# IGLICT/NeRFFaceEditing

Hardware: NVIDIA B200
Metric: rendered rays/sec (48+48 samples) (higher is better)
Workload: dtype f32 (gather, compositing) + bf16x3 split tensor-core MLP with f32 accumulate

## Files before the change

### include/nfe_b200.h

```cpp
#ifndef NFE_B200_H
#define NFE_B200_H

#include <stdint.h>

#ifdef __cplusplus
extern "C" {
#endif

typedef void* nfe_stream_t;

int nfe_version(void);
const char* nfe_last_error(void);
uint64_t nfe_launch_count(void);
int nfe_timing_enable(int on);
int nfe_timing_read(double* ms_by_stage, int64_t* count_by_stage, int n_stages, int reset);

int nfe_bench_l2_gather(const float* table, int64_t n_lines, int warps_per_cta, int depth, int iters, int64_t* host_lines_out,
                        float* sink, nfe_stream_t stream);

int nfe_plane_stats(const float* planes, int64_t n_slabs, int64_t hw, float* mean, float* std_out,
                    nfe_stream_t stream);
int nfe_plane_normalize(const float* planes, const float* mean, const float* std_in, int64_t n_slabs,
                        int64_t hw, float* out, nfe_stream_t stream);
int nfe_plane_denormalize(const float* norm, const float* mean, const float* std_in, int64_t n_slabs,
                          int64_t stat_slabs, int64_t hw, float* out, nfe_stream_t stream);
int nfe_plane_normalize_bwd(const float* g_norm, const float* norm, const float* std_in, const float* g_mean,
                            const float* g_std, int64_t n_slabs, int64_t hw, double* sums_ws, float* g_planes,
                            nfe_stream_t stream);
int nfe_resize_bilinear(const float* in, int64_t n_img, int in_h, int in_w, int out_h, int out_w, int antialias,
                        float* out, nfe_stream_t stream);
int nfe_planes_to_channel_last(const float* planes, int64_t n_img, int channels, int64_t hw, float* out,
                               nfe_stream_t stream);

int nfe_plane_normalize_staged(const float* planes, const float* mean, const float* std_in, int64_t n_img,
                               int64_t hw, float* out_norm, float* out_norm_cl, float* out_raw_cl,
                               nfe_stream_t stream);

int nfe_generate_rays(const float* cam2world , const float* intrinsics , int n,
                      int resolution, float* origins , float* dirs, nfe_stream_t stream);
int nfe_ray_limits_box(const float* origins, const float* dirs, int64_t n_rays, float box_side_length,
                       float* tmin, float* tmax, nfe_stream_t stream);

int nfe_sample_stratified(int64_t n_rays, int s_c, int mode, const float* table, double ray_start,
                          double ray_end, const float* start_per_ray, const float* end_per_ray,
                          const float* jitter, int stochastic, uint64_t seed, uint64_t offset,
                          float* depths , nfe_stream_t stream);

int nfe_sample_planes_fwd(const float* planes_cl, int plane_batch, int channels, int height, int width,
                          const float* coords , int n, int64_t m, float box_warp, float* out,
                          nfe_stream_t stream);

// ... 144 lines not shown
```

### nerffaceediting_b200/_lib.py

```python
import ctypes
import os

_HERE = os.path.dirname(os.path.abspath(__file__))
LIB_PATH = os.path.join(_HERE, "lib", "libnfe_b200.so")

DEC_OSG, DEC_DISENTANGLED, DEC_SEGMENTATION = 0, 1, 2
PREC_FP32, PREC_BF16X3, PREC_BF16 = 0, 1, 2

c_f32p = ctypes.c_void_p
c_i64 = ctypes.c_int64
c_u64 = ctypes.c_uint64
c_int = ctypes.c_int
c_float = ctypes.c_float
c_double = ctypes.c_double
c_vp = ctypes.c_void_p


class NfeMlp(ctypes.Structure):
    _fields_ = [("w1", c_vp), ("b1", c_vp), ("w2", c_vp), ("b2", c_vp),
                ("in_dim", c_int), ("hidden", c_int), ("out_dim", c_int),
                ("wgain1", c_float), ("bgain1", c_float), ("wgain2", c_float), ("bgain2", c_float)]


class NfeRenderCfg(ctypes.Structure):
# ... 12 lines not shown


_MLP_P = ctypes.POINTER(NfeMlp)
_CFG_P = ctypes.POINTER(NfeRenderCfg)

SIGNATURES = {
    "nfe_version": (c_int, []),
    "nfe_last_error": (ctypes.c_char_p, []),
    "nfe_launch_count": (c_u64, []),
    "nfe_timing_enable": (c_int, [c_int]),
    "nfe_timing_read": (c_int, [ctypes.POINTER(c_double), ctypes.POINTER(c_i64), c_int, c_int]),
    "nfe_bench_l2_gather": (c_int, [c_vp, c_i64, c_int, c_int, c_int, ctypes.POINTER(c_i64), c_vp, c_vp]),
    "nfe_plane_stats": (c_int, [c_vp, c_i64, c_i64, c_vp, c_vp, c_vp]),
    "nfe_plane_normalize": (c_int, [c_vp, c_vp, c_vp, c_i64, c_i64, c_vp, c_vp]),
    "nfe_plane_denormalize": (c_int, [c_vp, c_vp, c_vp, c_i64, c_i64, c_i64, c_vp, c_vp]),
    "nfe_plane_normalize_staged": (c_int, [c_vp, c_vp, c_vp, c_i64, c_i64, c_vp, c_vp, c_vp, c_vp]),
    "nfe_planes_to_channel_last": (c_int, [c_vp, c_i64, c_int, c_i64, c_vp, c_vp]),
    "nfe_generate_rays": (c_int, [c_vp, c_vp, c_int, c_int, c_vp, c_vp, c_vp]),
    "nfe_ray_limits_box": (c_int, [c_vp, c_vp, c_i64, c_float, c_vp, c_vp, c_vp]),
    "nfe_sample_stratified": (c_int, [c_i64, c_int, c_int, c_vp, c_double, c_double, c_vp, c_vp, c_vp, c_int, c_u64, c_u64, c_vp, c_vp]),
    "nfe_sample_planes_fwd": (c_int, [c_vp, c_int, c_int, c_int, c_int, c_vp, c_int, c_i64, c_float, c_vp, c_vp]),
    "nfe_decoder_fwd": (c_int, [c_int, c_int, _MLP_P, _MLP_P, c_vp, c_vp, c_int, c_i64, c_int, c_vp, c_vp, c_vp, c_vp]),
    "nfe_composite_fwd": (c_int, [c_vp, c_vp, c_vp, c_vp, c_i64, c_int, c_int, c_int, c_int, c_vp, c_vp, c_vp, c_vp, c_vp, c_vp, c_vp]),
    "nfe_importance_resample": (c_int, [c_vp, c_vp, c_i64, c_int, c_int, c_vp, c_int, c_u64, c_u64, c_vp, c_vp, c_vp, c_vp]),
    "nfe_sample_pdf": (c_int, [c_vp, c_vp, c_i64, c_int, c_int, c_int, c_vp, c_int, c_u64, c_u64, c_float, c_vp, c_vp]),
    "nfe_unify_samples":(c_int, [c_vp] * 8 + [c_i64, c_int, c_int, c_int, c_int] + [c_vp] * 4 + [c_vp]),
    "nfe_render_workspace_bytes": (c_i64, [_CFG_P, c_int, c_i64]),
    "nfe_render_fwd": (c_int, [_CFG_P, _MLP_P, _MLP_P, c_vp, c_vp, c_int, c_vp, c_vp, c_int, c_i64, c_vp, c_vp,
                               c_vp, c_vp, c_vp, c_vp, c_vp, c_int, c_vp, c_vp, c_vp, c_i64, c_vp]),
    "nfe_render_workspace_layout": (c_int, [_CFG_P, c_int, c_i64, ctypes.POINTER(c_i64)]),
    "nfe_composite_bwd": (c_int, [c_vp, c_vp, c_vp, c_int, c_vp, c_vp, c_vp, c_int, c_i64, c_int, c_int, c_vp, c_vp, c_vp, c_vp, c_vp, c_vp, c_vp, c_vp]),
# ... 66 lines not shown
```

### nerffaceediting_b200/autograd.py

```python
import ctypes
import os

import torch
import torch.nn.functional as F

from . import _lib, ops

MAX_ROWS = 1 << 22


def _mlp(x, seq):
    a, b = seq[0], seq[2]
    h = F.softplus(torch.addmm((a.bias * a.bias_gain).unsqueeze(0), x, (a.weight * a.weight_gain).t()))
    return torch.addmm((b.bias * b.bias_gain).unsqueeze(0), h, (b.weight * b.weight_gain).t())


def _decode(kind, seq_a, seq_b, fn, fd):
    if kind == ops.DEC_DISENTANGLED:
        g = _mlp(fn, seq_a)
        return g[:, :1], g[:, 1:], torch.sigmoid(_mlp(fd, seq_b)) * (1 + 2 * 0.001) - 0.001
    x = _mlp(fd, seq_a)
    rgb = torch.sigmoid(x[:, 1:]) * (1 + 2 * 0.001) - 0.001
    return x[:, :1], (_mlp(fd, seq_b) if kind == ops.DEC_SEGMENTATION else None), rgb

# ... 210 lines not shown
        if g.get("rgb") is not None:
            g_rec[:, 16:48] = g["rgb"].reshape(n * m, 32)
        with torch.cuda.device(dev):
            fb = _FieldBackward(kind, seq_a, seq_b, norm_cl, denorm_cl, ctx.affine, ctx.box_warp, ctx.needs_input_grad[5:], dev)
            fb.run_pass(n, rec, g_rec, coords=coords)
            norm_shape, plane_shape = ctx.plane_shapes
            g_norm, g_planes, g_scale, g_shift, g_params = fb.finish(norm_shape, plane_shape, ctx.needs_input_grad[1], ctx.needs_input_grad[2],
                                                                     ctx.stat_shapes, ctx.needs_input_grad[3], ctx.needs_input_grad[4])
        return (None, g_norm, g_planes, g_scale, g_shift) + tuple(g_params)


class NormalizeFunction(torch.autograd.Function):

    @staticmethod
    def forward(ctx, planes):
        mean, std = ops.plane_stats(planes)
        norm_cl = None
        if planes.dim() == 4 and planes.shape[1] == 96 and planes.is_contiguous() and planes.dtype == torch.float32:
            norm, norm_cl, _ = ops.plane_normalize_staged(planes.detach(), mean, std, register=False)
        else:
            norm = ops.plane_normalize(planes, mean, std)
        ctx.save_for_backward(norm, std)
        ctx.hw = planes.shape[-1] * planes.shape[-2]
        if norm_cl is None:
            return norm, mean, std, None
        ctx.mark_non_differentiable(norm_cl)
        return norm, mean, std, norm_cl

    @staticmethod
    def backward(ctx, g_norm, g_mean, g_std, _g_cl=None):
        norm, std = ctx.saved_tensors
        def f32(t):
            return None if t is None else t.contiguous().float()
        g, gm, gs = f32(g_norm), f32(g_mean), f32(g_std)
        slabs = norm.numel() // ctx.hw
# ... 30 lines not shown
```

### nerffaceediting_b200/csrc/nfe_march.cu

```cuda
#include "nfe_march.cuh"

namespace nfe {

__device__ __forceinline__ double shfl_up_double(double v, int delta)
{
    int lo = __double2loint(v), hi = __double2hiint(v);
    lo = __shfl_up_sync(0xffffffffu, lo, delta);
    hi = __shfl_up_sync(0xffffffffu, hi, delta);
    return __hiloint2double(hi, lo);
}
__device__ __forceinline__ double shfl_xor_double(double v, int mask)
{
    int lo = __double2loint(v), hi = __double2hiint(v);
    lo = __shfl_xor_sync(0xffffffffu, lo, mask);
    hi = __shfl_xor_sync(0xffffffffu, hi, mask);
    return __hiloint2double(hi, lo);
}

__device__ __forceinline__ void ray_interval_weights(const float* s_depth, const float* s_sigma, float* s_w, int S, int lane, float& wd, float& wt)
{
    const int n_int = S - 1;
    const int chunk = (n_int + 31) / 32;
    const int i0 = lane * chunk, i1 = min(n_int, i0 + chunk);
    float prod = 1.0f;
    for (int i = i0; i < i1; ++i) {
        const float delta = __fsub_rn(s_depth[i + 1], s_depth[i]);
        const float sig = __fdiv_rn(__fadd_rn(s_sigma[i], s_sigma[i + 1]), 2.0f);
        const float xs = __fsub_rn(sig, 1.0f);
        const float dens = fmaxf(xs, 0.0f) + __logf(1.0f + __expf(-fabsf(xs)));
        const float alpha = __fsub_rn(1.0f, __expf(-__fmul_rn(dens, delta)));
        s_w[i] = alpha;
        prod *= __fadd_rn(__fsub_rn(1.0f, alpha), 1e-10f);
    }
    float incl = prod;
#pragma unroll
    for (int o = 1; o < 32; o <<= 1) {
        const float up = __shfl_up_sync(0xffffffffu, incl, o);
        if (lane >= o) incl *= up;
    }
    float T = __shfl_up_sync(0xffffffffu, incl, 1);
    if (lane == 0) T = 1.0f;
    for (int i = i0; i < i1; ++i) {
        const float alpha = s_w[i];
        const float w = __fmul_rn(alpha, T);
        T *= __fadd_rn(__fsub_rn(1.0f, alpha), 1e-10f);
        s_w[i] = w;
        wd = fmaf(w, __fdiv_rn(__fadd_rn(s_depth[i], s_depth[i + 1]), 2.0f), wd);
        wt = __fadd_rn(wt, w);
    }
}

__device__ __forceinline__ void cp_async16(uint32_t dst_smem, const void* src)
{
    asm volatile("cp.async.cg.shared.global [%0], [%1], 16;" ::"r"(dst_smem), "l"(src) : "memory");
}
__device__ __forceinline__ void cp_async_commit() { asm volatile("cp.async.commit_group;" ::: "memory"); }
template <int N>
__device__ __forceinline__ void cp_async_wait() { asm volatile("cp.async.wait_group %0;" ::"n"(N) : "memory"); }

constexpr int MARCH_RING_GROUPS = 4;
constexpr int MARCH_MIN_BLOCKS = 4;
template <bool SORT>
// ... 248 lines not shown
            depths_out[ray * S + k] = s_d[e];
            sigma_out[ray * S + k] = e < a.s1 ? a.sigma1[ray * a.s1 + e] : a.sigma2[ray * a.s2 + (e - a.s1)];
        }
        for (int k = 0; k < S; ++k) {
            const int e = s_order[k];
            const bool first = e < a.s1;
            const int64_t row = first ? ray * a.s1 + e : ray * a.s2 + (e - a.s1);
            for (int c = lane; c < a.cc; c += 32) colors_out[(ray * S + k) * a.cc + c] = (first ? a.colors1 : a.colors2)[row * a.cc + c];
            for (int c = lane; c < a.cs; c += 32) segs_out[(ray * S + k) * a.cs + c] = (first ? a.segs1 : a.segs2)[row * a.cs + c];
        }
        __syncwarp();
    }
}

constexpr int RESAMPLE_MIN_BLOCKS = 4;
template <bool SMOOTH>
__global__ void __launch_bounds__(256, RESAMPLE_MIN_BLOCKS) resample_kernel(ResampleArgs a)
{
    extern __shared__ __align__(16) float smem[];
    const int warp = threadIdx.x >> 5, lane = threadIdx.x & 31;
    const int warps_per_block = blockDim.x >> 5;
    const int S = a.S, nw = S - 1, ns = SMOOTH ? S - 3 : a.ns;
    const int per_warp = 4 * S + (a.sort_u ? a.s_f : 0);
    float* s_z = smem + (size_t)warp * per_warp;
    float* s_om = s_z + S;
    float* s_bins = s_om + S;
    float* s_cdf = s_bins + S;
    float* s_u = s_cdf + S;
    for (int64_t ray = (int64_t)blockIdx.x * warps_per_block + warp; ray < a.n_rays; ray += (int64_t)gridDim.x * warps_per_block) {
        if (SMOOTH) {
            for (int e = lane; e < S; e += 32) s_z[e] = a.z_vals[ray * S + e];
            if (a.sigma) {
                for (int e = lane; e < S; e += 32) s_om[e] = a.sigma[ray * S + e];
                __syncwarp();
                float wd = 0.0f, wt = 0.0f;
                ray_interval_weights(s_z, s_om, s_cdf, S, lane, wd, wt);
                __syncwarp();
                if (a.weights_out) for (int e = lane; e < nw; e += 32) a.weights_out[ray * nw + e] = s_cdf[e];
            } else {
                for (int e = lane; e < nw; e += 32) s_cdf[e] = a.weights[ray * nw + e];
            }
            __syncwarp();
            for (int i = lane; i < nw; i += 32) {
                const float w0 = s_cdf[i];
                const float m_i = i > 0 ? fmaxf(s_cdf[i - 1], w0) : w0;
                const float m_n = i + 1 < nw ? fmaxf(w0, s_cdf[i + 1]) : w0;
                const float sm = __fadd_rn(__fdiv_rn(__fadd_rn(m_i, m_n), 2.0f), 0.01f);
                if (i >= 1 && i <= ns) s_om[i - 1] = __fadd_rn(sm, a.eps);
                s_bins[i] = __fmul_rn(0.5f, __fadd_rn(s_z[i], s_z[i + 1]));
            }
        } else {
            for (int e = lane; e < S; e += 32) s_bins[e] = a.z_vals[ray * S + e];
            for (int e = lane; e < ns; e += 32) s_om[e] = __fadd_rn(a.weights[ray * ns + e], a.eps);
        }
        __syncwarp();
        double tot = 0.0;
        for (int j = lane; j < ns; j += 32) tot += (double)s_om[j];
#pragma unroll
        for (int o = 16; o > 0; o >>= 1) tot += shfl_xor_double(tot, o);
        const float totf = (float)tot;
        const int chunk = (ns + 31) / 32;
        const int j0 = lane * chunk, j1 = min(ns, j0 + chunk);
// ... 198 lines not shown
```

### nerffaceediting_b200/csrc/nfe_planes.cu

```cuda
#include "nfe_common.cuh"

namespace nfe {

__global__ void __launch_bounds__(512) plane_stats_kernel(const float* __restrict__ planes, int64_t hw,
                                                          float* __restrict__ mean, float* __restrict__ std_out)
{
    const float* x = planes + (int64_t)blockIdx.x * hw;
    double s = 0.0, ss = 0.0;
    const bool vec = (hw % 4 == 0) && ((reinterpret_cast<uintptr_t>(x) & 15) == 0);
    if (vec) {
        const float4* x4 = reinterpret_cast<const float4*>(x);
        const int64_t n4 = hw / 4;
        for (int64_t i = threadIdx.x; i < n4; i += blockDim.x) {
            const float4 v = __ldg(x4 + i);
            s += (double)v.x; s += (double)v.y; s += (double)v.z; s += (double)v.w;
            ss += (double)v.x * (double)v.x; ss += (double)v.y * (double)v.y;
            ss += (double)v.z * (double)v.z; ss += (double)v.w * (double)v.w;
        }
    } else {
        for (int64_t i = threadIdx.x; i < hw; i += blockDim.x) {
            const double v = (double)x[i];
            s += v; ss += v * v;
        }
    }
#pragma unroll
    for (int o = 16; o > 0; o >>= 1) {
        s += __shfl_xor_sync(0xffffffffu, s, o);
        ss += __shfl_xor_sync(0xffffffffu, ss, o);
    }
    __shared__ double sh_s[16], sh_ss[16];
    const int warp = threadIdx.x >> 5, lane = threadIdx.x & 31;
    if (lane == 0) { sh_s[warp] = s; sh_ss[warp] = ss; }
    __syncthreads();
    if (warp == 0) {
        const int nw = blockDim.x >> 5;
        s = lane < nw ? sh_s[lane] : 0.0;
        ss = lane < nw ? sh_ss[lane] : 0.0;
#pragma unroll
        for (int o = 8; o > 0; o >>= 1) {
            s += __shfl_xor_sync(0xffffffffu, s, o);
            ss += __shfl_xor_sync(0xffffffffu, ss, o);
        }
        if (lane == 0) {
            const double n = (double)hw;
            const double m = s / n;
            double var = (ss - s * m) / (n - 1.0);
            if (var < 0.0) var = 0.0;
            mean[blockIdx.x] = (float)m;
            std_out[blockIdx.x] = sqrtf((float)var);
        }
    }
}

__global__ void __launch_bounds__(256) plane_normalize_kernel(const float* __restrict__ planes, const float* __restrict__ mean,
                                                              const float* __restrict__ std_in, int64_t hw, int chunks_per_slab,
                                                              float* __restrict__ out)
{
    const int64_t slab = blockIdx.x / chunks_per_slab;
    const int chunk = blockIdx.x % chunks_per_slab;
    const float m = mean[slab];
    const float d = __fadd_rn(std_in[slab], 1e-8f);
    const int64_t per = (hw + chunks_per_slab - 1) / chunks_per_slab;
    const int64_t lo = chunk * per, hi = min(hw, lo + per);
    const float* x = planes + slab * hw;
    float* y = out + slab * hw;
    const bool vec = (hw % 4 == 0) && (per % 4 == 0) && (((reinterpret_cast<uintptr_t>(x) | reinterpret_cast<uintptr_t>(y)) & 15) == 0);
// ... 48 lines not shown
    const float* src = planes + img * channels * hw;
    float* dst = out + img * hw * channels;
    const int npx = (int)min((int64_t)CL_PIX, hw - px0);
    for (int i = threadIdx.x; i < channels * CL_PIX; i += blockDim.x) {
        const int c = i / CL_PIX, p = i % CL_PIX;
        if (p < npx) tile[c * (CL_PIX + 1) + p] = __ldg(src + (int64_t)c * hw + px0 + p);
    }
    __syncthreads();
    for (int i = threadIdx.x; i < npx * channels; i += blockDim.x) {
        const int p = i / channels, c = i % channels;
        dst[(px0 + p) * channels + c] = tile[c * (CL_PIX + 1) + p];
    }
}

constexpr int STAGE_MIN_BLOCKS = 4;
template <bool NORMALIZE>
__global__ void __launch_bounds__(256, STAGE_MIN_BLOCKS) stage32_kernel(const float* __restrict__ planes, const float* __restrict__ mean,
                                                      const float* __restrict__ std_in, int64_t hw, int64_t groups_per_img, int64_t n_groups,
                                                      float* __restrict__ out_norm, float* __restrict__ out_norm_cl, float* __restrict__ out_raw_cl)
{
    const int lane = threadIdx.x & 31;
    int64_t group = ((int64_t)blockIdx.x * blockDim.x + threadIdx.x) >> 5;
    if (group >= n_groups) return;
    if constexpr (NORMALIZE) group = n_groups - 1 - group;
    const int64_t img = group / groups_per_img;
    const int64_t px = (group % groups_per_img) * 32 + lane;
    const bool live = px < hw;
    const float* src = planes + img * 32 * hw + px;
    float x[32];
#pragma unroll
    for (int c = 0; c < 32; ++c) x[c] = live ? __ldg(src + (int64_t)c * hw) : 0.0f;
    if (live && out_raw_cl) {
        float4* dst = reinterpret_cast<float4*>(out_raw_cl + (img * hw + px) * 32);
#pragma unroll
        for (int q = 0; q < 8; ++q) dst[q] = make_float4(x[4 * q], x[4 * q + 1], x[4 * q + 2], x[4 * q + 3]);
    }
    if constexpr (NORMALIZE) {
        const float m_l = mean[img * 32 + lane];
        const float d_l = __fadd_rn(std_in[img * 32 + lane], 1e-8f);
#pragma unroll
        for (int c = 0; c < 32; ++c) {
            const float m = __shfl_sync(0xffffffffu, m_l, c), d = __shfl_sync(0xffffffffu, d_l, c);
            x[c] = __fdiv_rn(__fsub_rn(x[c], m), d);
        }
        if (live) {
            float* dn = out_norm + img * 32 * hw + px;
#pragma unroll
            for (int c = 0; c < 32; ++c) __stcs(dn + (int64_t)c * hw, x[c]);
            float4* dst = reinterpret_cast<float4*>(out_norm_cl + (img * hw + px) * 32);
#pragma unroll
            for (int q = 0; q < 8; ++q) dst[q] = make_float4(x[4 * q], x[4 * q + 1], x[4 * q + 2], x[4 * q + 3]);
        }
    }
}


__global__ void __launch_bounds__(512) plane_normalize_bwd_sums_kernel(const float* __restrict__ g, const float* __restrict__ norm, int64_t hw,
                                                                       double* __restrict__ sums)
{
    const float* gp = g + (int64_t)blockIdx.x * hw;
    const float* np_ = norm + (int64_t)blockIdx.x * hw;
    double s = 0.0, sn = 0.0;
    const bool vec = (hw % 4 == 0) && (((reinterpret_cast<uintptr_t>(gp) | reinterpret_cast<uintptr_t>(np_)) & 15) == 0);
    if (vec) {
        const float4* g4 = reinterpret_cast<const float4*>(gp);
        const float4* n4 = reinterpret_cast<const float4*>(np_);
        for (int64_t i = threadIdx.x; i < hw / 4; i += blockDim.x) {
// ... 119 lines not shown
{
    int64_t c = (int64_t)sm_count() * 16 / (n_slabs > 0 ? n_slabs : 1);
    const int64_t max_c = hw / 4096 > 0 ? hw / 4096 : 1;
    if (c > max_c) c = max_c;
    if (c < 1) c = 1;
    while (c > 1 && ((hw % c) != 0 || ((hw / c) % 4) != 0)) --c;
    return (int)c;
}

NFE_EXPORT int nfe_plane_stats(const float* planes, int64_t n_slabs, int64_t hw, float* mean, float* std_out, nfe_stream_t stream)
{
    if (n_slabs == 0) return 0;
    NFE_REQUIRE(planes && mean && std_out, "nfe_plane_stats: null pointer");
    NFE_REQUIRE(n_slabs >= 0 && n_slabs < (1ll << 31) && hw >= 2, "nfe_plane_stats: bad sizes (n_slabs=%lld hw=%lld)", (long long)n_slabs, (long long)hw);
    if (n_slabs == 0) return 0;
    plane_stats_kernel<<<(unsigned)n_slabs, 512, 0, as_stream(stream)>>>(planes, hw, mean, std_out);
    NFE_LAUNCH_CHECK("plane_stats_kernel");
    return 0;
}

NFE_EXPORT int nfe_plane_normalize(const float* planes, const float* mean, const float* std_in, int64_t n_slabs, int64_t hw,
                                   float* out, nfe_stream_t stream)
{
    if (n_slabs == 0 || hw == 0) return 0;
    NFE_REQUIRE(planes && mean && std_in && out, "nfe_plane_normalize: null pointer");
    NFE_REQUIRE(n_slabs >= 0 && hw >= 1, "nfe_plane_normalize: bad sizes");
    if (n_slabs == 0) return 0;
    const int chunks = chunks_for(n_slabs, hw);
    NFE_REQUIRE(n_slabs * chunks < (1ll << 31), "nfe_plane_normalize: grid too large");
    plane_normalize_kernel<<<(unsigned)(n_slabs * chunks), 256, 0, as_stream(stream)>>>(planes, mean, std_in, hw, chunks, out);
    NFE_LAUNCH_CHECK("plane_normalize_kernel");
// ... 11 lines not shown
    NFE_REQUIRE(n_slabs * chunks < (1ll << 31), "nfe_plane_denormalize: grid too large");
    plane_denormalize_kernel<<<(unsigned)(n_slabs * chunks), 256, 0, as_stream(stream)>>>(norm, mean, std_in, stat_slabs, hw, chunks, out);
    NFE_LAUNCH_CHECK("plane_denormalize_kernel");
    return 0;
}

NFE_EXPORT int nfe_planes_to_channel_last(const float* planes, int64_t n_img, int channels, int64_t hw, float* out, nfe_stream_t stream)
{
    if (n_img == 0 || hw == 0) return 0;
    NFE_REQUIRE(planes && out, "nfe_planes_to_channel_last: null pointer");
    NFE_REQUIRE(n_img >= 0 && channels >= 1 && channels <= 256 && hw >= 1, "nfe_planes_to_channel_last: bad sizes");
    if (n_img == 0) return 0;
    if (channels == 32 && (reinterpret_cast<uintptr_t>(out) & 15) == 0) {
        const int64_t groups_per_img = (hw + 31) / 32, n_groups = n_img * groups_per_img;
        NFE_REQUIRE((n_groups + 7) / 8 < (1ll << 31), "nfe_planes_to_channel_last: grid too large");
        stage32_kernel<false><<<(unsigned)((n_groups + 7) / 8), 256, 0, as_stream(stream)>>>(planes, nullptr, nullptr, hw, groups_per_img, n_groups,
                                                                                           nullptr, nullptr, out);
        NFE_LAUNCH_CHECK("stage32_kernel");
        return 0;
    }
    const int64_t tiles = (hw + CL_PIX - 1) / CL_PIX;
    NFE_REQUIRE(n_img * tiles < (1ll << 31), "nfe_planes_to_channel_last: grid too large");
    const size_t smem = (size_t)channels * (CL_PIX + 1) * sizeof(float);
    if (smem > 48 * 1024) cudaFuncSetAttribute(to_channel_last_kernel, cudaFuncAttributeMaxDynamicSharedMemorySize, (int)smem);
    to_channel_last_kernel<<<(unsigned)(n_img * tiles), 256, smem, as_stream(stream)>>>(planes, channels, hw, tiles, out);
    NFE_LAUNCH_CHECK("to_channel_last_kernel");
    return 0;
}

NFE_EXPORT int nfe_plane_normalize_staged(const float* planes, const float* mean, const float* std_in, int64_t n_img, int64_t hw, float* out_norm,
                                          float* out_norm_cl, float* out_raw_cl, nfe_stream_t stream)
{
    if (n_img == 0 || hw == 0) return 0;
    NFE_REQUIRE(planes && mean && std_in && out_norm && out_norm_cl, "nfe_plane_normalize_staged: null pointer");
    NFE_REQUIRE(((reinterpret_cast<uintptr_t>(out_norm_cl) | reinterpret_cast<uintptr_t>(out_raw_cl)) & 15) == 0,
                "nfe_plane_normalize_staged: channel-last outputs must be 16-byte aligned");
    const int64_t groups_per_img = (hw + 31) / 32, n_groups = n_img * groups_per_img;
    NFE_REQUIRE((n_groups + 7) / 8 < (1ll << 31), "nfe_plane_normalize_staged: grid too large");
    stage32_kernel<true><<<(unsigned)((n_groups + 7) / 8), 256, 0, as_stream(stream)>>>(planes, mean, std_in, hw, groups_per_img, n_groups, out_norm,
                                                                                      out_norm_cl, out_raw_cl);
    NFE_LAUNCH_CHECK("stage32_kernel");
    return 0;
}

NFE_EXPORT int nfe_plane_normalize_bwd(const float* g_norm, const float* norm, const float* std_in, const float* g_mean, const float* g_std,
                                       int64_t n_slabs, int64_t hw, double* sums_ws, float* g_planes, nfe_stream_t stream)
{
    if (n_slabs == 0 || hw == 0) return 0;
    NFE_REQUIRE(norm && std_in && g_planes, "nfe_plane_normalize_bwd: null pointer");
    NFE_REQUIRE(!g_norm || sums_ws, "nfe_plane_normalize_bwd: the reduction workspace ([n_slabs,2] doubles) is missing");
    NFE_REQUIRE(n_slabs >= 0 && hw >= 2, "nfe_plane_normalize_bwd: bad sizes");
    NFE_REQUIRE(n_slabs < (1ll << 31), "nfe_plane_normalize_bwd: grid too large");
    if (g_norm) {
        plane_normalize_bwd_sums_kernel<<<(unsigned)n_slabs, 512, 0, as_stream(stream)>>>(g_norm, norm, hw, sums_ws);
        NFE_LAUNCH_CHECK("plane_normalize_bwd_sums_kernel");
    }
    const int chunks = chunks_for(n_slabs, hw);
// ... 20 lines not shown
```

### nerffaceediting_b200/ops.py

```python
import ctypes

import os

import torch

from . import _lib
from . import plane_registry as registry
from ._lib import DEC_DISENTANGLED, DEC_OSG, DEC_SEGMENTATION, NfeMlp, NfeRenderCfg


def _cuda_f32(t, name):
    if not isinstance(t, torch.Tensor):
        raise RuntimeError(f"{name}: expected a tensor, got {type(t).__name__}")
    if not t.is_cuda:
        raise RuntimeError(f"{name}: expected a CUDA tensor (this path has no CPU fallback), got device {t.device}")
    if t.dtype != torch.float32:
        t = t.float()
    return t.contiguous()


def _ptr(t):
    return None if t is None else t.data_ptr()


# ... 103 lines not shown
    x = _cuda_f32(planes, "planes")
    if x.dim() != 5 or x.shape[1] != 3:
        raise RuntimeError(f"planes: expected [N,3,C,H,W], got {tuple(x.shape)}")
    hit = registry.staged_get(x)
    if hit is not None:
        return hit
    n, p, c, h, w = x.shape
    out = torch.empty((n, p, h, w, c), device=x.device, dtype=torch.float32)
    with _Guard(x):
        _lib.check(_lib.load().nfe_planes_to_channel_last(_ptr(x), n * p, c, h * w, _ptr(out), _stream(x)), "nfe_planes_to_channel_last")
    if cache and x is planes:
        registry.staged_put(planes, out)
    return out


def plane_normalize_staged(planes, mean, std, stage_raw=False, register=True):
    x = _cuda_f32(planes, "planes")
    n, c96, h, w = x.shape
    norm = torch.empty_like(x)
    norm_cl = torch.empty((n, 3, h, w, 32), device=x.device, dtype=torch.float32)
    raw_cl = torch.empty_like(norm_cl) if stage_raw else None
    with _Guard(x):
        _lib.check(_lib.load().nfe_plane_normalize_staged(_ptr(x), _ptr(mean), _ptr(std), n * 3, h * w, _ptr(norm), _ptr(norm_cl), _ptr(raw_cl),
                                                          _stream(x)), "nfe_plane_normalize_staged")
    if register:
        register_normalized(planes, norm, mean, std, norm_cl, raw_cl)
    return norm, norm_cl, raw_cl


def register_normalized(planes, norm, mean, std, norm_cl, raw_cl=None):
    n = planes.shape[0]
    registry.staged_put(norm, norm_cl)
    if raw_cl is not None:
        registry.staged_put(planes, raw_cl)
    registry.provenance_put(planes, norm, std.detach().reshape(n, -1) + 1e-8, mean.detach().reshape(n, -1))


def clear_plane_cache():
    registry.clear()


def generate_rays(cam2world, intrinsics, resolution):
# ... 381 lines not shown
```

### nerffaceediting_b200/triplane.py

```python
import numpy as np
import torch

from . import ops


class FullyConnectedLayer(torch.nn.Module):

    def __init__(self, in_features, out_features, bias=True, activation='linear', lr_multiplier=1, bias_init=0):
        super().__init__()
        assert activation == 'linear' and bias, "only the linear, biased layer of the decoders is provided"
        self.in_features = in_features
        self.out_features = out_features
        self.activation = activation
        self.weight = torch.nn.Parameter(torch.randn([out_features, in_features]) / lr_multiplier)
        self.bias = torch.nn.Parameter(torch.full([out_features], np.float32(bias_init)))
        self.weight_gain = lr_multiplier / np.sqrt(in_features)
        self.bias_gain = lr_multiplier

    def extra_repr(self):
        return f'in_features={self.in_features:d}, out_features={self.out_features:d}, activation={self.activation:s}'


def _mlp(n_features, hidden, out, lr_mul):
    return torch.nn.Sequential(FullyConnectedLayer(n_features, hidden, lr_multiplier=lr_mul), torch.nn.Softplus(),
# ... 40 lines not shown

def compute_mean_var(planes):
    ops._no_grad_needed(planes)
    return ops.plane_stats(planes)


def normalize_plane(planes):
    tri = planes.dim() == 4 and planes.shape[1] == 96 and planes.is_contiguous() and planes.dtype == torch.float32
    if torch.is_grad_enabled() and planes.requires_grad:
        from .autograd import NormalizeFunction
        norm, mean, std, norm_cl = NormalizeFunction.apply(planes)
        if norm_cl is not None:
            ops.register_normalized(planes, norm, mean, std, norm_cl)
            ops.provenance_attach(planes, std, 1e-8, mean)
        return norm, mean, std
    mean, std = ops.plane_stats(planes)
    if tri:
        return ops.plane_normalize_staged(planes, mean, std)[0], mean, std
    return ops.plane_normalize(planes, mean, std), mean, std


def denormalize_plane(planes, mean, var):
    if torch.is_grad_enabled() and any(torch.is_tensor(t) and t.requires_grad for t in (planes, mean, var)):
        from .autograd import DenormalizeFunction
        out = DenormalizeFunction.apply(planes, mean, var)
        if torch.is_tensor(mean) and torch.is_tensor(var):
            ops.register_denormalized(out, planes, mean, var)
            ops.provenance_attach(out, var, 0.0, mean, norm_requires_grad=planes.requires_grad)
        return out
    return ops.plane_denormalize(planes, mean, var)


class TriPlaneGenerator(torch.nn.Module):
# ... 97 lines not shown
```

Baseline: 34.01 million.

## Fuse plane stats and normalize/stage into one persistent ticketed kernel

Replaces the separate plane-stats and normalize-staging launches with one persistent kernel. Blocks take tasks from an atomic ticket counter, with stats tasks for each group of images ordered ahead of their staging tasks and a per-item done counter with acquire spin-wait. Stats reads use L2 evict_last hints so staging can re-read the planes from L2, and stats loads are batched for more memory-level parallelism. The resample kernel also prefetches the next ray's depths and sigmas into registers, and divisions by two become multiplications by a half. The persistent counters are cached per device, stream and shape, which adds complexity and a risk of deadlock or ordering bugs.

```diff
diff --git a/include/nfe_b200.h b/include/nfe_b200.h
--- a/include/nfe_b200.h
+++ b/include/nfe_b200.h
@@ -32,9 +32,9 @@
 int nfe_planes_to_channel_last(const float* planes, int64_t n_img, int channels, int64_t hw, float* out,
                                nfe_stream_t stream);
 
-int nfe_plane_normalize_staged(const float* planes, const float* mean, const float* std_in, int64_t n_img,
-                               int64_t hw, float* out_norm, float* out_norm_cl, float* out_raw_cl,
-                               nfe_stream_t stream);
+int nfe_plane_prep(const float* planes, int64_t n_img, int64_t hw, float* mean, float* std_out, float* out_norm,
+                   float* out_norm_cl, float* out_raw_cl, int64_t* counters, nfe_stream_t stream);
+int64_t nfe_plane_prep_task_order(int64_t n_img, int64_t hw, int64_t cap, int32_t* stage, int64_t* item, int64_t* sub);
 
 int nfe_generate_rays(const float* cam2world , const float* intrinsics , int n,
                       int resolution, float* origins , float* dirs, nfe_stream_t stream);
diff --git a/nerffaceediting_b200/_lib.py b/nerffaceediting_b200/_lib.py
--- a/nerffaceediting_b200/_lib.py
+++ b/nerffaceediting_b200/_lib.py
@@ -50,7 +50,8 @@
     "nfe_plane_stats": (c_int, [c_vp, c_i64, c_i64, c_vp, c_vp, c_vp]),
     "nfe_plane_normalize": (c_int, [c_vp, c_vp, c_vp, c_i64, c_i64, c_vp, c_vp]),
     "nfe_plane_denormalize": (c_int, [c_vp, c_vp, c_vp, c_i64, c_i64, c_i64, c_vp, c_vp]),
-    "nfe_plane_normalize_staged": (c_int, [c_vp, c_vp, c_vp, c_i64, c_i64, c_vp, c_vp, c_vp, c_vp]),
+    "nfe_plane_prep": (c_int, [c_vp, c_i64, c_i64, c_vp, c_vp, c_vp, c_vp, c_vp, c_vp, c_vp]),
+    "nfe_plane_prep_task_order": (c_i64, [c_i64, c_i64, c_i64, c_vp, c_vp, c_vp]),
     "nfe_planes_to_channel_last": (c_int, [c_vp, c_i64, c_int, c_i64, c_vp, c_vp]),
     "nfe_generate_rays": (c_int, [c_vp, c_vp, c_int, c_int, c_vp, c_vp, c_vp]),
     "nfe_ray_limits_box": (c_int, [c_vp, c_vp, c_i64, c_float, c_vp, c_vp, c_vp]),
diff --git a/nerffaceediting_b200/autograd.py b/nerffaceediting_b200/autograd.py
--- a/nerffaceediting_b200/autograd.py
+++ b/nerffaceediting_b200/autograd.py
@@ -248,11 +248,11 @@
 
     @staticmethod
     def forward(ctx, planes):
-        mean, std = ops.plane_stats(planes)
         norm_cl = None
         if planes.dim() == 4 and planes.shape[1] == 96 and planes.is_contiguous() and planes.dtype == torch.float32:
-            norm, norm_cl, _ = ops.plane_normalize_staged(planes.detach(), mean, std, register=False)
+            norm, mean, std, norm_cl, _ = ops.plane_prep(planes.detach(), register=False)
         else:
+            mean, std = ops.plane_stats(planes)
             norm = ops.plane_normalize(planes, mean, std)
         ctx.save_for_backward(norm, std)
         ctx.hw = planes.shape[-1] * planes.shape[-2]
diff --git a/nerffaceediting_b200/csrc/nfe_march.cu b/nerffaceediting_b200/csrc/nfe_march.cu
--- a/nerffaceediting_b200/csrc/nfe_march.cu
+++ b/nerffaceediting_b200/csrc/nfe_march.cu
@@ -25,7 +25,7 @@
     float prod = 1.0f;
     for (int i = i0; i < i1; ++i) {
         const float delta = __fsub_rn(s_depth[i + 1], s_depth[i]);
-        const float sig = __fdiv_rn(__fadd_rn(s_sigma[i], s_sigma[i + 1]), 2.0f);
+        const float sig = __fmul_rn(__fadd_rn(s_sigma[i], s_sigma[i + 1]), 0.5f);
         const float xs = __fsub_rn(sig, 1.0f);
         const float dens = fmaxf(xs, 0.0f) + __logf(1.0f + __expf(-fabsf(xs)));
         const float alpha = __fsub_rn(1.0f, __expf(-__fmul_rn(dens, delta)));
@@ -45,7 +45,7 @@
         const float w = __fmul_rn(alpha, T);
         T *= __fadd_rn(__fsub_rn(1.0f, alpha), 1e-10f);
         s_w[i] = w;
-        wd = fmaf(w, __fdiv_rn(__fadd_rn(s_depth[i], s_depth[i + 1]), 2.0f), wd);
+        wd = fmaf(w, __fmul_rn(__fadd_rn(s_depth[i], s_depth[i + 1]), 0.5f), wd);
         wt = __fadd_rn(wt, w);
     }
 }
@@ -324,6 +324,7 @@
 }
 
 constexpr int RESAMPLE_MIN_BLOCKS = 4;
+constexpr int RESAMPLE_PREFETCH = 2;
 template <bool SMOOTH>
 __global__ void __launch_bounds__(256, RESAMPLE_MIN_BLOCKS) resample_kernel(ResampleArgs a)
 {
@@ -337,17 +338,37 @@
     float* s_bins = s_om + S;
     float* s_cdf = s_bins + S;
     float* s_u = s_cdf + S;
-    for (int64_t ray = (int64_t)blockIdx.x * warps_per_block + warp; ray < a.n_rays; ray += (int64_t)gridDim.x * warps_per_block) {
+    const int64_t ray_step = (int64_t)gridDim.x * warps_per_block;
+    float pf_z[RESAMPLE_PREFETCH], pf_s[RESAMPLE_PREFETCH];
+    auto prefetch = [&](int64_t r) {
+#pragma unroll
+        for (int j = 0; j < RESAMPLE_PREFETCH; ++j) {
+            const int e = lane + 32 * j;
+            const bool on = SMOOTH && r < a.n_rays && e < S;
+            pf_z[j] = on ? a.z_vals[r * S + e] : 0.0f;
+            pf_s[j] = on && a.sigma ? a.sigma[r * S + e] : 0.0f;
+        }
+    };
+    prefetch((int64_t)blockIdx.x * warps_per_block + warp);
+    for (int64_t ray = (int64_t)blockIdx.x * warps_per_block + warp; ray < a.n_rays; ray += ray_step) {
         if (SMOOTH) {
-            for (int e = lane; e < S; e += 32) s_z[e] = a.z_vals[ray * S + e];
+#pragma unroll
+            for (int j = 0; j < RESAMPLE_PREFETCH; ++j)
+                if (lane + 32 * j < S) s_z[lane + 32 * j] = pf_z[j];
+            for (int e = lane + 32 * RESAMPLE_PREFETCH; e < S; e += 32) s_z[e] = a.z_vals[ray * S + e];
             if (a.sigma) {
-                for (int e = lane; e < S; e += 32) s_om[e] = a.sigma[ray * S + e];
+#pragma unroll
+                for (int j = 0; j < RESAMPLE_PREFETCH; ++j)
+                    if (lane + 32 * j < S) s_om[lane + 32 * j] = pf_s[j];
+                for (int e = lane + 32 * RESAMPLE_PREFETCH; e < S; e += 32) s_om[e] = a.sigma[ray * S + e];
+                prefetch(ray + ray_step);
                 __syncwarp();
                 float wd = 0.0f, wt = 0.0f;
                 ray_interval_weights(s_z, s_om, s_cdf, S, lane, wd, wt);
                 __syncwarp();
                 if (a.weights_out) for (int e = lane; e < nw; e += 32) a.weights_out[ray * nw + e] = s_cdf[e];
             } else {
+                prefetch(ray + ray_step);
                 for (int e = lane; e < nw; e += 32) s_cdf[e] = a.weights[ray * nw + e];
             }
             __syncwarp();
@@ -355,7 +376,7 @@
                 const float w0 = s_cdf[i];
                 const float m_i = i > 0 ? fmaxf(s_cdf[i - 1], w0) : w0;
                 const float m_n = i + 1 < nw ? fmaxf(w0, s_cdf[i + 1]) : w0;
-                const float sm = __fadd_rn(__fdiv_rn(__fadd_rn(m_i, m_n), 2.0f), 0.01f);
+                const float sm = __fadd_rn(__fmul_rn(__fadd_rn(m_i, m_n), 0.5f), 0.01f);
                 if (i >= 1 && i <= ns) s_om[i - 1] = __fadd_rn(sm, a.eps);
                 s_bins[i] = __fmul_rn(0.5f, __fadd_rn(s_z[i], s_z[i + 1]));
             }
diff --git a/nerffaceediting_b200/csrc/nfe_planes.cu b/nerffaceediting_b200/csrc/nfe_planes.cu
--- a/nerffaceediting_b200/csrc/nfe_planes.cu
+++ b/nerffaceediting_b200/csrc/nfe_planes.cu
@@ -2,24 +2,59 @@
 
 namespace nfe {
 
-__global__ void __launch_bounds__(512) plane_stats_kernel(const float* __restrict__ planes, int64_t hw,
-                                                          float* __restrict__ mean, float* __restrict__ std_out)
-{
-    const float* x = planes + (int64_t)blockIdx.x * hw;
+__device__ __forceinline__ uint64_t l2_policy_evict_last()
+{
+    uint64_t p;
+    asm("createpolicy.fractional.L2::evict_last.b64 %0, 1.0;" : "=l"(p));
+    return p;
+}
+__device__ __forceinline__ uint64_t l2_policy_evict_first()
+{
+    uint64_t p;
+    asm("createpolicy.fractional.L2::evict_first.b64 %0, 1.0;" : "=l"(p));
+    return p;
+}
+__device__ __forceinline__ float4 ldg_hint(const float4* p, uint64_t pol)
+{
+    float4 v;
+    asm("ld.global.nc.L2::cache_hint.v4.f32 {%0, %1, %2, %3}, [%4], %5;" : "=f"(v.x), "=f"(v.y), "=f"(v.z), "=f"(v.w) : "l"(p), "l"(pol));
+    return v;
+}
+__device__ __forceinline__ float ldg_hint(const float* p, uint64_t pol)
+{
+    float v;
+    asm("ld.global.nc.L2::cache_hint.f32 %0, [%1], %2;" : "=f"(v) : "l"(p), "l"(pol));
+    return v;
+}
+
+constexpr int STATS_THREADS = 512;
+constexpr int STATS_BATCH = 4;
+template <bool HINT>
+__device__ __forceinline__ void slab_stats(const float* __restrict__ x, int64_t hw, uint64_t pol, float* __restrict__ mean,
+                                           float* __restrict__ std_out)
+{
     double s = 0.0, ss = 0.0;
     const bool vec = (hw % 4 == 0) && ((reinterpret_cast<uintptr_t>(x) & 15) == 0);
     if (vec) {
         const float4* x4 = reinterpret_cast<const float4*>(x);
         const int64_t n4 = hw / 4;
-        for (int64_t i = threadIdx.x; i < n4; i += blockDim.x) {
-            const float4 v = __ldg(x4 + i);
+        auto add = [&](const float4 v) {
             s += (double)v.x; s += (double)v.y; s += (double)v.z; s += (double)v.w;
             ss += (double)v.x * (double)v.x; ss += (double)v.y * (double)v.y;
             ss += (double)v.z * (double)v.z; ss += (double)v.w * (double)v.w;
-        }
+        };
+        int64_t i = threadIdx.x;
+        for (; i + (STATS_BATCH - 1) * STATS_THREADS < n4; i += STATS_BATCH * STATS_THREADS) {
+            float4 v[STATS_BATCH];
+#pragma unroll
+            for (int u = 0; u < STATS_BATCH; ++u) v[u] = HINT ? ldg_hint(x4 + i + u * STATS_THREADS, pol) : __ldg(x4 + i + u * STATS_THREADS);
+#pragma unroll
+            for (int u = 0; u < STATS_BATCH; ++u) add(v[u]);
+        }
+        for (; i < n4; i += STATS_THREADS) add(HINT ? ldg_hint(x4 + i, pol) : __ldg(x4 + i));
     } else {
-        for (int64_t i = threadIdx.x; i < hw; i += blockDim.x) {
-            const double v = (double)x[i];
+        for (int64_t i = threadIdx.x; i < hw; i += STATS_THREADS) {
+            const double v = (double)(HINT ? ldg_hint(x + i, pol) : __ldg(x + i));
             s += v; ss += v * v;
         }
     }
@@ -33,7 +68,7 @@
     if (lane == 0) { sh_s[warp] = s; sh_ss[warp] = ss; }
     __syncthreads();
     if (warp == 0) {
-        const int nw = blockDim.x >> 5;
+        constexpr int nw = STATS_THREADS >> 5;
         s = lane < nw ? sh_s[lane] : 0.0;
         ss = lane < nw ? sh_ss[lane] : 0.0;
 #pragma unroll
@@ -46,10 +81,16 @@
             const double m = s / n;
             double var = (ss - s * m) / (n - 1.0);
             if (var < 0.0) var = 0.0;
-            mean[blockIdx.x] = (float)m;
-            std_out[blockIdx.x] = sqrtf((float)var);
-        }
-    }
+            *mean = (float)m;
+            *std_out = sqrtf((float)var);
+        }
+    }
+}
+
+__global__ void __launch_bounds__(STATS_THREADS) plane_stats_kernel(const float* __restrict__ planes, int64_t hw,
+                                                                   float* __restrict__ mean, float* __restrict__ std_out)
+{
+    slab_stats<false>(planes + (int64_t)blockIdx.x * hw, hw, 0, mean + blockIdx.x, std_out + blockIdx.x);
 }
 
 __global__ void __launch_bounds__(256) plane_normalize_kernel(const float* __restrict__ planes, const float* __restrict__ mean,
@@ -128,43 +169,119 @@
 }
 
 constexpr int STAGE_MIN_BLOCKS = 4;
-template <bool NORMALIZE>
-__global__ void __launch_bounds__(256, STAGE_MIN_BLOCKS) stage32_kernel(const float* __restrict__ planes, const float* __restrict__ mean,
-                                                      const float* __restrict__ std_in, int64_t hw, int64_t groups_per_img, int64_t n_groups,
-                                                      float* __restrict__ out_norm, float* __restrict__ out_norm_cl, float* __restrict__ out_raw_cl)
+__global__ void __launch_bounds__(256, STAGE_MIN_BLOCKS) stage32_kernel(const float* __restrict__ planes, int64_t hw, int64_t groups_per_img,
+                                                                       int64_t n_groups, float* __restrict__ out_raw_cl)
 {
     const int lane = threadIdx.x & 31;
-    int64_t group = ((int64_t)blockIdx.x * blockDim.x + threadIdx.x) >> 5;
+    const int64_t group = ((int64_t)blockIdx.x * blockDim.x + threadIdx.x) >> 5;
     if (group >= n_groups) return;
-    if constexpr (NORMALIZE) group = n_groups - 1 - group;
     const int64_t img = group / groups_per_img;
     const int64_t px = (group % groups_per_img) * 32 + lane;
-    const bool live = px < hw;
+    if (px >= hw) return;
     const float* src = planes + img * 32 * hw + px;
     float x[32];
 #pragma unroll
-    for (int c = 0; c < 32; ++c) x[c] = live ? __ldg(src + (int64_t)c * hw) : 0.0f;
-    if (live && out_raw_cl) {
-        float4* dst = reinterpret_cast<float4*>(out_raw_cl + (img * hw + px) * 32);
-#pragma unroll
-        for (int q = 0; q < 8; ++q) dst[q] = make_float4(x[4 * q], x[4 * q + 1], x[4 * q + 2], x[4 * q + 3]);
-    }
-    if constexpr (NORMALIZE) {
-        const float m_l = mean[img * 32 + lane];
-        const float d_l = __fadd_rn(std_in[img * 32 + lane], 1e-8f);
-#pragma unroll
-        for (int c = 0; c < 32; ++c) {
-            const float m = __shfl_sync(0xffffffffu, m_l, c), d = __shfl_sync(0xffffffffu, d_l, c);
-            x[c] = __fdiv_rn(__fsub_rn(x[c], m), d);
-        }
-        if (live) {
-            float* dn = out_norm + img * 32 * hw + px;
-#pragma unroll
-            for (int c = 0; c < 32; ++c) __stcs(dn + (int64_t)c * hw, x[c]);
-            float4* dst = reinterpret_cast<float4*>(out_norm_cl + (img * hw + px) * 32);
-#pragma unroll
-            for (int q = 0; q < 8; ++q) dst[q] = make_float4(x[4 * q], x[4 * q + 1], x[4 * q + 2], x[4 * q + 3]);
-        }
+    for (int c = 0; c < 32; ++c) x[c] = __ldg(src + (int64_t)c * hw);
+    float4* dst = reinterpret_cast<float4*>(out_raw_cl + (img * hw + px) * 32);
+#pragma unroll
+    for (int q = 0; q < 8; ++q) dst[q] = make_float4(x[4 * q], x[4 * q + 1], x[4 * q + 2], x[4 * q + 3]);
+}
+
+constexpr int PREP_THREADS = STATS_THREADS;
+constexpr int PREP_IMGS_PER_ITEM = 3;
+constexpr int PREP_STATS_TASKS = PREP_IMGS_PER_ITEM * 32;
+constexpr int PREP_STAGE_GROUPS = 4 * (PREP_THREADS / 32);
+constexpr int PREP_MIN_BLOCKS = 2;
+
+struct PrepTask { int stage; int64_t item, sub; };
+
+__host__ __device__ inline PrepTask prep_task(int64_t t, int64_t n_items, int64_t stage_tasks)
+{
+    if (t < PREP_STATS_TASKS) return {0, 0, t};
+    t -= PREP_STATS_TASKS;
+    const int64_t pair = PREP_STATS_TASKS + stage_tasks;
+    const int64_t p = 1 + t / pair, r = t % pair;
+    if (p < n_items && r < PREP_STATS_TASKS) return {0, p, r};
+    return {1, p - 1, p < n_items ? r - PREP_STATS_TASKS : r};
+}
+
+__global__ void __launch_bounds__(PREP_THREADS, PREP_MIN_BLOCKS)
+plane_prep_kernel(const float* __restrict__ planes, int64_t n_img, int64_t hw, float* mean, float* std_out, float* __restrict__ out_norm,
+                  float* __restrict__ out_norm_cl, float* __restrict__ out_raw_cl, unsigned long long* counters)
+{
+    const int warp = threadIdx.x >> 5, lane = threadIdx.x & 31;
+    const int64_t groups_per_img = (hw + 31) / 32;
+    const int64_t n_items = (n_img + PREP_IMGS_PER_ITEM - 1) / PREP_IMGS_PER_ITEM;
+    const int64_t stage_tasks = (PREP_IMGS_PER_ITEM * groups_per_img + PREP_STAGE_GROUPS - 1) / PREP_STAGE_GROUPS;
+    const unsigned long long n_tasks = (unsigned long long)(n_items * (PREP_STATS_TASKS + stage_tasks));
+    const unsigned long long per_call = n_tasks + gridDim.x;
+    unsigned long long* ticket_ctr = counters;
+    unsigned long long* done = counters + 1;
+    const uint64_t pol_keep = l2_policy_evict_last(), pol_drop = l2_policy_evict_first();
+    __shared__ unsigned long long sh_ticket;
+    for (;;) {
+        if (threadIdx.x == 0) sh_ticket = atomicAdd(ticket_ctr, 1ull);
+        __syncthreads();
+        const unsigned long long ticket = sh_ticket;
+        const unsigned long long epoch = ticket / per_call, t = ticket % per_call;
+        if (t >= n_tasks) return;
+        const PrepTask task = prep_task((int64_t)t, n_items, stage_tasks);
+        const int64_t img0 = task.item * PREP_IMGS_PER_ITEM;
+        const int64_t imgs = min((int64_t)PREP_IMGS_PER_ITEM, n_img - img0);
+        if (!task.stage) {
+            if (task.sub < imgs * 32) {
+                const int64_t slab = img0 * 32 + task.sub;
+                slab_stats<true>(planes + slab * hw, hw, pol_keep, mean + slab, std_out + slab);
+                if (threadIdx.x == 0) {
+                    __threadfence();
+                    atomicAdd(done + task.item, 1ull);
+                }
+            }
+        } else {
+            if (threadIdx.x == 0) {
+                const unsigned long long target = (epoch + 1) * (unsigned long long)(imgs * 32);
+                for (;;) {
+                    unsigned long long v;
+                    asm volatile("ld.acquire.gpu.global.u64 %0, [%1];" : "=l"(v) : "l"(done + task.item) : "memory");
+                    if (v >= target) break;
+                    __nanosleep(256);
+                }
+            }
+            __syncthreads();
+            const int64_t item_groups = imgs * groups_per_img;
+            for (int i = 0; i < PREP_STAGE_GROUPS / (PREP_THREADS / 32); ++i) {
+                const int64_t g = task.sub * PREP_STAGE_GROUPS + i * (PREP_THREADS / 32) + warp;
+                if (g >= item_groups) break;
+                const int64_t img = img0 + g / groups_per_img;
+                const int64_t px = (g % groups_per_img) * 32 + lane;
+                const bool live = px < hw;
+                const float* src = planes + img * 32 * hw + px;
+                float x[32];
+#pragma unroll
+                for (int c = 0; c < 32; ++c) x[c] = live ? ldg_hint(src + (int64_t)c * hw, pol_drop) : 0.0f;
+                if (live && out_raw_cl) {
+                    float4* dst = reinterpret_cast<float4*>(out_raw_cl + (img * hw + px) * 32);
+#pragma unroll
+                    for (int q = 0; q < 8; ++q) dst[q] = make_float4(x[4 * q], x[4 * q + 1], x[4 * q + 2], x[4 * q + 3]);
+                }
+                const float m_l = __ldcg(mean + img * 32 + lane);
+                const float d_l = __fadd_rn(__ldcg(std_out + img * 32 + lane), 1e-8f);
+#pragma unroll
+                for (int c = 0; c < 32; ++c) {
+                    const float m = __shfl_sync(0xffffffffu, m_l, c), d = __shfl_sync(0xffffffffu, d_l, c);
+                    x[c] = __fdiv_rn(__fsub_rn(x[c], m), d);
+                }
+                if (live) {
+                    float* dn = out_norm + img * 32 * hw + px;
+#pragma unroll
+                    for (int c = 0; c < 32; ++c) __stcs(dn + (int64_t)c * hw, x[c]);
+                    float4* dst = reinterpret_cast<float4*>(out_norm_cl + (img * hw + px) * 32);
+#pragma unroll
+                    for (int q = 0; q < 8; ++q) dst[q] = make_float4(x[4 * q], x[4 * q + 1], x[4 * q + 2], x[4 * q + 3]);
+                }
+            }
+        }
+        __syncthreads();
     }
 }
 
@@ -314,7 +431,7 @@
     NFE_REQUIRE(planes && mean && std_out, "nfe_plane_stats: null pointer");
     NFE_REQUIRE(n_slabs >= 0 && n_slabs < (1ll << 31) && hw >= 2, "nfe_plane_stats: bad sizes (n_slabs=%lld hw=%lld)", (long long)n_slabs, (long long)hw);
     if (n_slabs == 0) return 0;
-    plane_stats_kernel<<<(unsigned)n_slabs, 512, 0, as_stream(stream)>>>(planes, hw, mean, std_out);
+    plane_stats_kernel<<<(unsigned)n_slabs, STATS_THREADS, 0, as_stream(stream)>>>(planes, hw, mean, std_out);
     NFE_LAUNCH_CHECK("plane_stats_kernel");
     return 0;
 }
@@ -356,8 +473,7 @@
     if (channels == 32 && (reinterpret_cast<uintptr_t>(out) & 15) == 0) {
         const int64_t groups_per_img = (hw + 31) / 32, n_groups = n_img * groups_per_img;
         NFE_REQUIRE((n_groups + 7) / 8 < (1ll << 31), "nfe_planes_to_channel_last: grid too large");
-        stage32_kernel<false><<<(unsigned)((n_groups + 7) / 8), 256, 0, as_stream(stream)>>>(planes, nullptr, nullptr, hw, groups_per_img, n_groups,
-                                                                                           nullptr, nullptr, out);
+        stage32_kernel<<<(unsigned)((n_groups + 7) / 8), 256, 0, as_stream(stream)>>>(planes, hw, groups_per_img, n_groups, out);
         NFE_LAUNCH_CHECK("stage32_kernel");
         return 0;
     }
@@ -370,19 +486,38 @@
     return 0;
 }
 
-NFE_EXPORT int nfe_plane_normalize_staged(const float* planes, const float* mean, const float* std_in, int64_t n_img, int64_t hw, float* out_norm,
-                                          float* out_norm_cl, float* out_raw_cl, nfe_stream_t stream)
+NFE_EXPORT int nfe_plane_prep(const float* planes, int64_t n_img, int64_t hw, float* mean, float* std_out, float* out_norm, float* out_norm_cl,
+                              float* out_raw_cl, int64_t* counters, nfe_stream_t stream)
 {
     if (n_img == 0 || hw == 0) return 0;
-    NFE_REQUIRE(planes && mean && std_in && out_norm && out_norm_cl, "nfe_plane_normalize_staged: null pointer");
+    NFE_REQUIRE(planes && mean && std_out && out_norm && out_norm_cl && counters, "nfe_plane_prep: null pointer");
+    NFE_REQUIRE(n_img > 0 && hw >= 2, "nfe_plane_prep: bad sizes (n_img=%lld hw=%lld)", (long long)n_img, (long long)hw);
     NFE_REQUIRE(((reinterpret_cast<uintptr_t>(out_norm_cl) | reinterpret_cast<uintptr_t>(out_raw_cl)) & 15) == 0,
-                "nfe_plane_normalize_staged: channel-last outputs must be 16-byte aligned");
-    const int64_t groups_per_img = (hw + 31) / 32, n_groups = n_img * groups_per_img;
-    NFE_REQUIRE((n_groups + 7) / 8 < (1ll << 31), "nfe_plane_normalize_staged: grid too large");
-    stage32_kernel<true><<<(unsigned)((n_groups + 7) / 8), 256, 0, as_stream(stream)>>>(planes, mean, std_in, hw, groups_per_img, n_groups, out_norm,
-                                                                                      out_norm_cl, out_raw_cl);
-    NFE_LAUNCH_CHECK("stage32_kernel");
-    return 0;
+                "nfe_plane_prep: channel-last outputs must be 16-byte aligned");
+    const int64_t n_items = (n_img + PREP_IMGS_PER_ITEM - 1) / PREP_IMGS_PER_ITEM;
+    const int64_t stage_tasks = (PREP_IMGS_PER_ITEM * ((hw + 31) / 32) + PREP_STAGE_GROUPS - 1) / PREP_STAGE_GROUPS;
+    const int64_t n_tasks = n_items * (PREP_STATS_TASKS + stage_tasks);
+    int per_sm = 0;
+    const cudaError_t occ = cudaOccupancyMaxActiveBlocksPerMultiprocessor(&per_sm, plane_prep_kernel, PREP_THREADS, 0);
+    NFE_REQUIRE(occ == cudaSuccess, "nfe_plane_prep: occupancy query failed: %s", cudaGetErrorString(occ));
+    const int64_t resident = (int64_t)sm_count() * (per_sm > 0 ? per_sm : 1);
+    plane_prep_kernel<<<(unsigned)(n_tasks < resident ? n_tasks : resident), PREP_THREADS, 0, as_stream(stream)>>>(
+        planes, n_img, hw, mean, std_out, out_norm, out_norm_cl, out_raw_cl, reinterpret_cast<unsigned long long*>(counters));
+    NFE_LAUNCH_CHECK("plane_prep_kernel");
+    return 0;
+}
+
+NFE_EXPORT int64_t nfe_plane_prep_task_order(int64_t n_img, int64_t hw, int64_t cap, int32_t* stage, int64_t* item, int64_t* sub)
+{
+    if (n_img <= 0 || hw < 2) { set_error("nfe_plane_prep_task_order: bad sizes"); return -1; }
+    const int64_t n_items = (n_img + PREP_IMGS_PER_ITEM - 1) / PREP_IMGS_PER_ITEM;
+    const int64_t stage_tasks = (PREP_IMGS_PER_ITEM * ((hw + 31) / 32) + PREP_STAGE_GROUPS - 1) / PREP_STAGE_GROUPS;
+    const int64_t n_tasks = n_items * (PREP_STATS_TASKS + stage_tasks);
+    for (int64_t t = 0; t < n_tasks && t < cap; ++t) {
+        const PrepTask task = prep_task(t, n_items, stage_tasks);
+        stage[t] = task.stage; item[t] = task.item; sub[t] = task.sub;
+    }
+    return n_tasks;
 }
 
 NFE_EXPORT int nfe_plane_normalize_bwd(const float* g_norm, const float* norm, const float* std_in, const float* g_mean, const float* g_std,
diff --git a/nerffaceediting_b200/ops.py b/nerffaceediting_b200/ops.py
--- a/nerffaceediting_b200/ops.py
+++ b/nerffaceediting_b200/ops.py
@@ -141,18 +141,27 @@
     return out
 
 
-def plane_normalize_staged(planes, mean, std, stage_raw=False, register=True):
+_prep_counters = {}
+
+
+def plane_prep(planes, stage_raw=False, register=True):
     x = _cuda_f32(planes, "planes")
     n, c96, h, w = x.shape
+    mean = torch.empty((n, c96, 1, 1), device=x.device, dtype=torch.float32)
+    std = torch.empty_like(mean)
     norm = torch.empty_like(x)
     norm_cl = torch.empty((n, 3, h, w, 32), device=x.device, dtype=torch.float32)
     raw_cl = torch.empty_like(norm_cl) if stage_raw else None
+    key = (x.device.index, _stream(x), n, h * w)
+    counters = _prep_counters.get(key)
+    if counters is None:
+        counters = _prep_counters[key] = torch.zeros(1 + n, device=x.device, dtype=torch.int64)
     with _Guard(x):
-        _lib.check(_lib.load().nfe_plane_normalize_staged(_ptr(x), _ptr(mean), _ptr(std), n * 3, h * w, _ptr(norm), _ptr(norm_cl), _ptr(raw_cl),
-                                                          _stream(x)), "nfe_plane_normalize_staged")
+        _lib.check(_lib.load().nfe_plane_prep(_ptr(x), n * 3, h * w, _ptr(mean), _ptr(std), _ptr(norm), _ptr(norm_cl), _ptr(raw_cl),
+                                              _ptr(counters), _stream(x)), "nfe_plane_prep")
     if register:
         register_normalized(planes, norm, mean, std, norm_cl, raw_cl)
-    return norm, norm_cl, raw_cl
+    return norm, mean, std, norm_cl, raw_cl
 
 
 def register_normalized(planes, norm, mean, std, norm_cl, raw_cl=None):
diff --git a/nerffaceediting_b200/triplane.py b/nerffaceediting_b200/triplane.py
--- a/nerffaceediting_b200/triplane.py
+++ b/nerffaceediting_b200/triplane.py
@@ -78,9 +78,10 @@
             ops.register_normalized(planes, norm, mean, std, norm_cl)
             ops.provenance_attach(planes, std, 1e-8, mean)
         return norm, mean, std
+    if tri:
+        norm, mean, std, _, _ = ops.plane_prep(planes)
+        return norm, mean, std
     mean, std = ops.plane_stats(planes)
-    if tri:
-        return ops.plane_normalize_staged(planes, mean, std)[0], mean, std
     return ops.plane_normalize(planes, mean, std), mean, std
 
 
```

After: 34.00 million (median of 6 runs). About the same (-0.0%).
